# ViacheslavTimofeev/tpu_superresolution

Measured on AMD Instinct MI355X. Metric: HR pixels/sec, SwinIR x4 train step, 64x64 LR, bs=32/GPU, higher is better.
Workload: dtype bf16; 1 GPU; BASELINE cfg3: SwinIR classical x4 (dim 180, 6x6 blocks, window 8) train step = fwd + L1 + bwd + clip 1.0 + AdamW, 64x64 LR patches -> 256x256 HR, random-init weights, drop_path 0.1; every step starts from the seeded weights and fresh AdamW state; batch_per_gpu=32, global_batch=32, parallelism=dp1

## Files before the change

tpu_superresolution_amd/csrc/api.hip:

```cpp
#include <stdarg.h>
#include <stdio.h>
#include <string.h>

#include "adamw.h"
#include "kernels.h"
#include "tables.h"
#include "wgrad.h"

static thread_local char g_err[512] = "";

SrkOptTls& srk_opt_tls() {
  static thread_local SrkOptTls t = {};
  return t;
}

static SrkOpt** opt_table() {
  static SrkOpt* table[SRK_NUM_OPTS] = {};
  return table;
}

void srk_opt_register(SrkOpt* o) {
  if (o->id >= 0 && o->id < SRK_NUM_OPTS) opt_table()[o->id] = o;
}

// ... 320 lines not shown
  for (size_t i = 0; i < g_probe.count; ++i) {
    float t = 0.f;
    if (hipEventSynchronize(g_probe.ev1[i]) != hipSuccess || hipEventElapsedTime(&t, g_probe.ev0[i], g_probe.ev1[i]) != hipSuccess) {
      srk_set_error("probe_end: event query failed");
      return SRK_E_LAUNCH;
    }
    ms += t;
  }
  if (total_ms) *total_ms = ms;
  if (flops) *flops = g_probe.flops;
  if (bytes) *bytes = g_probe.bytes;
  if (launches) *launches = (int)g_probe.count;
  return SRK_OK;
}

namespace {

int tune_get(int which) {
  int v[4];
  srk_gemm_stream_tune_get(&v[0], &v[1], &v[2], &v[3]);
  return v[which];
}
int tune_set(int which, int value) {
  int v[4];
  srk_gemm_stream_tune_get(&v[0], &v[1], &v[2], &v[3]);
  v[which] = value;
  srk_gemm_stream_tune(v[0], v[1], v[2], v[3]);
  return SRK_OK;
}
int wtune_get(int which) {
  int rows, nt;
  srk_wgrad_stream_tune_get(&rows, &nt);
  return which == 0 ? rows : nt;
}

struct OptEntry {
  const char* name;
  int (*get)();
  int (*set)(int);
};

const OptEntry kOptions[] = {
    {"gemm_stream", [] { return srk_gemm_stream_enabled(); }, [](int v) { srk_gemm_stream_enable(v); return (int)SRK_OK; }},
    {"attn_bwd_fused", [] { return srk_attn_bwd_fused_enabled(); }, [](int v) { srk_attn_bwd_fused_enable(v); return (int)SRK_OK; }},
    {"attn_fused", [] { return srk_attn_fused_mode(); }, [](int v) { srk_attn_fused_enable(v); return (int)SRK_OK; }},
    {"wgrad_stream_w8", [] { return srk_wgrad_w8_enabled(); }, [](int v) { srk_wgrad_w8_enable(v); return (int)SRK_OK; }},
    {"block_light", [] { return srk_block_light_enabled(); }, [](int v) { srk_block_light_enable(v); return (int)SRK_OK; }},
    {"mlp_bwd_fused", [] { return srk_mlp_bwd_fused_enabled(); }, [](int v) { srk_mlp_bwd_fused_enable(v); return (int)SRK_OK; }},
    {"mlp_dgelu_store", [] { return srk_mlp_dgelu_store_enabled(); }, [](int v) { srk_mlp_dgelu_store_enable(v); return (int)SRK_OK; }},
    {"mlp_fused", [] { return srk_mlp_fused_enabled(); }, [](int v) { srk_mlp_fused_enable(v); return (int)SRK_OK; }},
    {"wgrad_stream", [] { return srk_wgrad_stream_enabled(); }, [](int v) { srk_wgrad_stream_enable(v); return (int)SRK_OK; }},
    {"conv_wgrad_taps", [] { return srk_conv_wgrad_taps_mode(); }, [](int v) { srk_conv_wgrad_taps_enable(v); return (int)SRK_OK; }},
    {"conv_wgrad_roll", [] { return srk_conv_wgrad_roll_enabled(); }, [](int v) { srk_conv_wgrad_roll_enable(v); return (int)SRK_OK; }},
    {"wgrad_partials", [] { return srk_wgrad_partials_enabled(); }, [](int v) { srk_wgrad_partials_enable(v); return (int)SRK_OK; }},
    {"wgrad_stream_rows", [] { return wtune_get(0); },
     [](int v) {
       SRK_REQUIRE(v == 32 || v == 64, SRK_E_SHAPE, "wgrad_stream_rows: 32/64");
       srk_wgrad_stream_tune(v, -1);
       return (int)SRK_OK;
     }},
    {"wgrad_stream_nt", [] { return wtune_get(1); }, [](int v) { srk_wgrad_stream_tune(0, v != 0); return (int)SRK_OK; }},
    {"gemm_stream_bm", [] { return tune_get(0); },
     [](int v) {
       SRK_REQUIRE(v == 0 || v == 16 || v == 32 || v == 64, SRK_E_SHAPE, "gemm_stream_bm: 0/16/32/64");
       return tune_set(0, v);
     }},
    {"gemm_stream_ks2", [] { return tune_get(1); }, [](int v) { return tune_set(1, v < 0 ? -1 : (v != 0)); }},
    {"gemm_stream_split", [] { return tune_get(2); }, [](int v) { return tune_set(2, v < 0 ? -1 : (v != 0)); }},
    {"gemm_stream_nb", [] { return tune_get(3); },
     [](int v) {
       SRK_REQUIRE(v == 0 || v == 4 || v == 8, SRK_E_SHAPE, "gemm_stream_nb: 0/4/8");
       return tune_set(3, v);
     }},
    {"probe_stride", [] { return g_probe.stride; },
     [](int v) {
       SRK_REQUIRE(v >= 1 && v <= 1024, SRK_E_SHAPE, "probe_stride: 1..1024");
       g_probe.stride = v;
       return (int)SRK_OK;
     }},
};

const OptEntry* find_option(const char* name) {
  for (const OptEntry& e : kOptions)
    if (strcmp(name, e.name) == 0) return &e;
  return nullptr;
}

}

int srk_set_option(const char* name, int value) {
  REQ_PTR(name);
  const OptEntry* e = find_option(name);
  if (!e) {
    srk_set_error("srk_set_option: unknown option '%s'", name);
    return SRK_E_UNSUPPORTED;
  }
  return e->set(value);
}

int srk_get_option(const char* name, int* value) {
  REQ_PTR(name); REQ_PTR(value);
  const OptEntry* e = find_option(name);
  if (!e) {
    srk_set_error("srk_get_option: unknown option '%s'", name);
    return SRK_E_UNSUPPORTED;
  }
// ... 402 lines not shown
```

tpu_superresolution_amd/csrc/common.h:

```cpp
#pragma once
#include <hip/hip_runtime.h>
#include <stdint.h>

#include "../../include/srk.h"

typedef unsigned short bf16_t;
typedef __attribute__((ext_vector_type(8))) short bf16x8_t;
typedef __attribute__((ext_vector_type(4))) short bf16x4_t;
typedef __attribute__((ext_vector_type(4))) float f32x4_t;

#define SRK_WAVE 64

void srk_set_error(const char* fmt, ...);
int srk_check_launch(const char* what);

constexpr int SRK_MAX_DEVICES = 64;
int srk_current_device();
int srk_device_cus();
enum SrkOptId {
  OPT_MLP_FUSED, OPT_MLP_BWD_FUSED, OPT_GEMM_STREAM, OPT_TUNE_BM, OPT_TUNE_KS2, OPT_TUNE_SPLIT, OPT_TUNE_NB, OPT_ATTN_BWD_FUSED,
  OPT_ATTN_FUSED, OPT_BLOCK_LIGHT, OPT_TAPS_ENABLED, OPT_TAPS_DMA, OPT_WGRAD_STREAM, OPT_WGRAD_ROWS, OPT_WGRAD_NT, OPT_WGRAD_W8,
  OPT_WGRAD_PARTIALS, OPT_MLP_DGELU_STORE, OPT_TAPS_ROLL, SRK_NUM_OPTS
};
struct SrkOptTls {
  int v[SRK_NUM_OPTS];
  unsigned on;
};
SrkOptTls& srk_opt_tls();
struct SrkOpt;
void srk_opt_register(SrkOpt* o);
void srk_opt_scope_begin(SrkOptTls* saved);
void srk_opt_scope_end(const SrkOptTls& saved);
struct SrkOpt {
  int id;
  int value;
  SrkOpt(int id_, int v) : id(id_), value(v) { srk_opt_register(this); }
  operator int() const {
    const SrkOptTls& t = srk_opt_tls();
    return ((t.on >> id) & 1u) ? t.v[id] : value;
  }
  SrkOpt& operator=(int v) {
    SrkOptTls& t = srk_opt_tls();
    if ((t.on >> id) & 1u) t.v[id] = v;
    else value = v;
    return *this;
  }
  SrkOpt(const SrkOpt&) = delete;
  SrkOpt& operator=(const SrkOpt&) = delete;
};

template <class T>
struct SrkPerDevice {
  T v[SRK_MAX_DEVICES] = {};
  T& here() { return v[srk_current_device()]; }
};

typedef SrkPerDevice<signed char> SrkLdsState;
int srk_reserve_lds_fn(const void* fn, int bytes, SrkLdsState& st, bool refuse_spills, const char* err_fmt, ...);
template <class K, class... A>
inline int srk_reserve_lds(K* kernel, size_t bytes, SrkLdsState& st, bool refuse_spills = false, const char* err_fmt = nullptr, A... a) {
  return srk_reserve_lds_fn(reinterpret_cast<const void*>(kernel), (int)bytes, st, refuse_spills, err_fmt, a...);
}

enum { FAM_GEMM_LINEAR = 1, FAM_GEMM_CONV = 2, FAM_WGRAD_LINEAR = 3, FAM_WGRAD_CONV = 4, FAM_ATTN_FWD = 5, FAM_ATTN_BWD = 6,
       FAM_LN = 7 };
void srk_probe_pre(int family, hipStream_t stream, double flops, double bytes = 0.0);
void srk_probe_post(int family, hipStream_t stream);

#define SRK_REQUIRE(cond, code, ...)      \
  do {                                    \
    if (!(cond)) {                        \
      srk_set_error(__VA_ARGS__);         \
      return (code);                      \
    }                                     \
  } while (0)
// ... 223 lines not shown
```

tpu_superresolution_amd/csrc/convwgrad.hip:

```cpp
#include <type_traits>

#include "wgrad.h"

#ifndef SRK_NT_TAPS
#define SRK_NT_TAPS 0
#endif

namespace {

constexpr int CT = 64;
constexpr int SP = 64 + 16;
constexpr int HALO = CT + 2;
constexpr int XROWS = 3 * HALO;
constexpr int YPIECES = CT * 8 / 256;
constexpr int XPIECES = (XROWS * 8 + 255) / 256;

template <bool SHUF>
__global__ __launch_bounds__(256) void conv_wgrad_taps_kernel(const WgradParams p, int ntiles, int chunks_per) {
  extern __shared__ __attribute__((aligned(16))) unsigned char smem[];
  bf16_t* Ys = reinterpret_cast<bf16_t*>(smem);
  bf16_t* Xs = Ys + 2 * CT * SP;

  const int tid = threadIdx.x, lane = tid & 63;
  const int wave = __builtin_amdgcn_readfirstlane(tid >> 6);
  const int r16 = lane & 15, g = lane >> 4;
  const int logical = xcd_remap(blockIdx.x, gridDim.x);
  const int bsplit = logical / ntiles, btile = logical - bsplit * ntiles;
  const int ntn = p.N / 64;
  const int tn = btile % ntn, tk = btile / ntn;
  const int n0 = tn * 64, k0 = tk * 64;
  const int c_begin = bsplit * chunks_per;
  const int c_end = min(p.M / CT, c_begin + chunks_per);
  if (c_begin >= c_end) return;
  const int hw = p.H * p.W;

  uint4 ry[YPIECES], rx[XPIECES];
  auto load_stage = [&](int ch) {
    const int m0 = ch * CT;
    const int b = m0 / hw, rem = m0 - b * hw;
    const int y = rem / p.W, x0 = rem - y * p.W;
#pragma unroll
    for (int t = 0; t < YPIECES; ++t) {
      const int pid = tid + 256 * t;
      const int row = pid >> 3, c8 = pid & 7;
      if constexpr (SHUF) {
        const int nn = n0 + c8 * 8;
        const int ij = nn / p.Cs, c = nn - ij * p.Cs;
        const int si = ij / p.r, sj = ij - si * p.r;
        ry[t] = *reinterpret_cast<const uint4*>(
            p.Y + (((long long)(b * p.H * p.r + y * p.r + si)) * (p.W * p.r) + (x0 + row) * p.r + sj) * p.Cs + c);
      } else {
        ry[t] = *reinterpret_cast<const uint4*>(p.Y + (long long)(m0 + row) * p.ldy + n0 + c8 * 8);
      }
    }
// ... 500 lines not shown
  const int cg = 9 * wave + q;
  const long long col = (long long)(cg >> 2) * p.K + tk * 64 + 16 * (cg & 3) + r16;
#pragma unroll
  for (int e = 0; e < 4; ++e) atomicAdd(p.dW + (long long)(n + e) * p.ldw + col, sum[e]);
}

SrkOpt g_taps_dma{OPT_TAPS_DMA, 1};
SrkOpt g_taps_roll{OPT_TAPS_ROLL, 1};

template <bool SHUF>
int launch_taps_dma(const WgradParams& p, hipStream_t stream) {
  constexpr int lds_staged = TD_RING * TD_STAGE_BYTES;
  constexpr int lds_roll = RL<2>::LDS > RL<1>::LDS ? RL<2>::LDS : RL<1>::LDS;
  static_assert(lds_roll <= 160 * 1024 && lds_staged <= 160 * 1024, "LDS budget");
  const int rpr = g_taps_roll && (p.W == CT || p.W == 2 * CT) && p.M % p.W == 0 ? p.W / CT : 0;
  static SrkLdsState reserved[2];
  constexpr const char* err = "conv wgrad (dma): cannot reserve %d bytes of LDS";
  constexpr int lds_max = lds_roll > lds_staged ? lds_roll : lds_staged;
  if (const int rc = rpr ? srk_reserve_lds(&conv_wgrad_taps_dma_kernel<SHUF>, lds_roll, reserved[1], false, err, lds_max)
                         : srk_reserve_lds(&conv_wgrad_taps_dma_staged_kernel<SHUF>, lds_staged, reserved[0], false, err, lds_max))
    return rc;
  const int lds = rpr == 1 ? RL<1>::LDS : (rpr == 2 ? RL<2>::LDS : lds_staged);
  const int unit = rpr ? rpr : 1;
  const int tiles = (p.N / 64) * (p.K / 64);
  const int nchunks = p.M / CT / unit;
  int splits = 256 / tiles;
  if (splits < 1) splits = 1;
  if (splits > nchunks) splits = nchunks;
  const int chunks_per = cdiv(nchunks, splits);
  splits = cdiv(nchunks, chunks_per);
  float* partial =
      srk_wgrad_partials_enabled() && splits > 1 ? srk_wgrad_scratch(stream, (size_t)tiles * splits * WS_SLAB_VEC * 16) : nullptr;
  srk_probe_pre(FAM_WGRAD_CONV, stream, p.flops, p.bytes);
  if (rpr)
    hipLaunchKernelGGL((conv_wgrad_taps_dma_kernel<SHUF>), dim3(tiles * splits), dim3(256), lds, stream, p, tiles, chunks_per * unit,
                       partial, splits, rpr);
  else
    hipLaunchKernelGGL((conv_wgrad_taps_dma_staged_kernel<SHUF>), dim3(tiles * splits), dim3(256), lds, stream, p, tiles, chunks_per,
                       partial, splits);
  if (partial) hipLaunchKernelGGL(conv_wgrad_taps_reduce_kernel, dim3(tiles * 36), dim3(256), 0, stream, p, partial, splits);
  srk_probe_post(FAM_WGRAD_CONV, stream);
  return srk_check_launch("conv wgrad (all taps, dma)");
}

__device__ __forceinline__ void split_bf16x8(const float (&v)[8], bf16x8_t& hi, bf16x8_t& lo) {
#pragma unroll
  for (int i = 0; i < 8; ++i) {
    const bf16_t h = f2bf(v[i]);
    hi[i] = (short)h;
    lo[i] = (short)f2bf(v[i] - bf2f(h));
  }
}

template <int COP>
struct SR {
  static constexpr int A = 3, NY = A + 1, NR = A + 3;
  static constexpr int GYB = CT * COP * 4;
  static constexpr int ROWB = HALO * 128;
  static constexpr int X_OFF = NY * GYB, Z_OFF = X_OFF + NR * ROWB, LDS = Z_OFF + ROWB;
};

template <bool NT = false>
__device__ __forceinline__ void srk_glds16_s1(const void* sb, unsigned voff, unsigned dst) {
  unsigned keep;
  asm volatile("s_mov_b32 %0, m0\n\ts_mov_b32 m0, %2\n\ts_nop 0\n\tglobal_load_lds_dwordx4 %1, %3\n\ts_mov_b32 m0, %0"
               : "=&s"(keep)
               : "v"(voff), "s"(dst), "s"(sb)
               : "memory");
}

__device__ __forceinline__ float lds_read_f32(unsigned addr) {
  return *reinterpret_cast<const float __attribute__((address_space(3)))*>(addr);
}

template <int COP>
__global__ __launch_bounds__(256, 2) void smallconv_wgrad_mfma_kernel(const bf16_t* __restrict__ x, const float* __restrict__ gy,
                                                                      float* __restrict__ dW, float* __restrict__ db, int B, int H, int W,
                                                                      int Cin, int CinP, int Co, int ntiles, int chunks_per) {
  using C = SR<COP>;
  extern __shared__ __attribute__((aligned(16))) unsigned char smem[];
  const unsigned lds0 = (unsigned)(size_t)smem;
  const int tid = threadIdx.x, lane = tid & 63;
  const int wave = __builtin_amdgcn_readfirstlane(tid >> 6);
  const int logical = xcd_remap(blockIdx.x, gridDim.x);
  const int bsplit = logical / ntiles, tk = logical - bsplit * ntiles;
  const int k0 = tk * 64;
  const int NCH = (int)(((long long)B * H * W) / CT);
  const int c_begin = bsplit * chunks_per;
  const int c_end = min(NCH, c_begin + chunks_per);
  if (c_begin >= c_end) return;
  const int nrun = c_end - c_begin;
  const int nxb = W / CT;
  for (int i = tid; i < HALO * 8; i += 256) *reinterpret_cast<uint4*>(smem + C::Z_OFF + i * 16) = make_uint4(0, 0, 0, 0);

  auto locate = [&](int ch, int& cy, int& cxb) -> long long {
    const int b = ch / (H * nxb), r = ch - b * (H * nxb);
    cxb = r / H;
    cy = r - cxb * H;
    return ((long long)(b * H + cy)) * W + cxb * CT;
  };
  auto step = [&](int& cy, int& cxb, const char*& ptr, long long ebytes) {
    if (++cy == H) {
      cy = 0;
      if (++cxb == nxb) {
        cxb = 0;
        ptr += CT * ebytes;
      } else {
        ptr += ((long long)CT - (long long)(H - 1) * W) * ebytes;
      }
    } else {
      ptr += (long long)W * ebytes;
    }
  };
  const long long xe = (long long)CinP * 2, ge = (long long)COP * 4;
  int xj = c_begin - 1, xy, xxb, gyy, gxb, y;
  const char* xptr = reinterpret_cast<const char*>(x + k0) + locate(max(xj, 0), xy, xxb) * xe;
  const char* gptr = reinterpret_cast<const char*>(gy) + locate(c_begin, gyy, gxb) * ge;
  y = gyy;
  const char* zero = reinterpret_cast<const char*>(g_zero_page);

  constexpr int LA = CT * COP / 16;
  const int l8 = lane >> 3, pos = lane & 7;
  const unsigned voffx = 2u * (unsigned)(l8 * CinP + ((((pos >> 1) ^ ((l8 >> 1) & 3)) << 1) | (pos & 1)) * 8);
  const unsigned voffh = (unsigned)(((wave & 1) * 4 + (lane & 3)) * 16);
  const unsigned voffg = (unsigned)((lane & (LA - 1)) * 16);
  const unsigned gdst0 = lds0 + (unsigned)(wave * LA * 16), gdst_end = gdst0 + C::NY * C::GYB;
  const unsigned xdst0 = lds0 + C::X_OFF, xdst_end = xdst0 + C::NR * C::ROWB;
  unsigned gdst = gdst0, xdst = xdst0;
  auto issue_y = [&]() {
    if (LA == 64 || lane < LA) srk_glds16_s1(gptr + wave * LA * 16, voffg, gdst);
    gdst = gdst + C::GYB == gdst_end ? gdst0 : gdst + C::GYB;
// ... 40 lines not shown
  for (int k = 0; k < C::A && k < nrun; ++k) {
    issue_y();
    issue_x();
  }
  const unsigned zrow = lds0 + C::Z_OFF;
  unsigned gs = lds0, xs0 = xdst0, xs1 = xdst0 + C::ROWB, xs2 = xdst0 + 2 * C::ROWB;
  auto run_loop = [&](auto bias) {
  constexpr bool BIAS = decltype(bias)::value;
  for (int it = 0; it < nrun; ++it) {
    if (it + C::A - 1 < nrun) srk_wait_vmcnt<4 * (C::A - 1)>(); else srk_wait_vmcnt<0>();
    srk_lds_barrier();
    if (it + C::A < nrun) {
      issue_y();
      issue_x();
    }
    const unsigned rb0 = y > 0 ? xs0 : zrow;
    const unsigned rb2 = y + 1 < H ? xs2 : zrow;
    const unsigned rbA = dA == 0 ? rb0 : (dA == 1 ? xs1 : rb2);
    const unsigned rbB = dB == 0 ? rb0 : (dB == 1 ? xs1 : rb2);
#pragma unroll
    for (int ks = 0; ks < 2; ++ks) {
      float v[8];
#pragma unroll
      for (int jj = 0; jj < 8; ++jj) {
        const float t = lds_read_f32(gs + goff + (unsigned)((32 * ks + 16 * (jj >> 2) + (jj & 3)) * COP * 4));
        v[jj] = ll < COP ? t : 0.f;
      }
      bf16x8_t yfh, yfl;
      split_bf16x8(v, yfh, yfl);
#pragma unroll
      for (int q = 0; q < 9; ++q) {
        const unsigned rb = q < nsel ? rbA : rbB;
        const bf16x4_t lo = lds_tr_read_at(ks == 0 ? rb + xoff0[q] : rb + (unsigned)xoff[q] + 32 * 128);
        const bf16x4_t hi = lds_tr_read_at(rb + (unsigned)xoff[q] + (32 * ks + 16) * 128);
        const bf16x8_t xf = bf16x8_t{lo[0], lo[1], lo[2], lo[3], hi[0], hi[1], hi[2], hi[3]};
        acc[q] = __builtin_amdgcn_mfma_f32_16x16x32_bf16(yfh, xf, acc[q], 0, 0, 0);
        acc[q] = __builtin_amdgcn_mfma_f32_16x16x32_bf16(yfl, xf, acc[q], 0, 0, 0);
      }
      if constexpr (BIAS) {
        accb = __builtin_amdgcn_mfma_f32_16x16x32_bf16(yfh, ones, accb, 0, 0, 0);
        accb = __builtin_amdgcn_mfma_f32_16x16x32_bf16(yfl, ones, accb, 0, 0, 0);
      }
    }
    gs = gs + C::GYB == lds0 + C::X_OFF ? lds0 : gs + C::GYB;
    xs0 = xs1;
    xs1 = xs2;
    xs2 = xs2 + C::ROWB == xdst_end ? xdst0 : xs2 + C::ROWB;
    y = y + 1 == H ? 0 : y + 1;
  }
  };
  if (do_bias) run_loop(std::true_type{});
  else run_loop(std::false_type{});

#pragma unroll
  for (int q = 0; q < 9; ++q) {
    const int cg = 9 * wave + q;
    const int tap = cg >> 2, k = k0 + 16 * (cg & 3) + ll;
#pragma unroll
    for (int e = 0; e < 4; ++e) {
      const int n = 4 * g + e;
      if (n < Co && k < Cin) atomicAdd(dW + ((long long)(n * Cin) + k) * 9 + tap, acc[q][e]);
    }
  }
  if (do_bias && ll == 0) {
#pragma unroll
    for (int e = 0; e < 4; ++e)
      if (4 * g + e < Co) atomicAdd(db + 4 * g + e, accb[e]);
  }
}

template <int COP>
__global__ __launch_bounds__(256) void smallconv_wgrad_mfma_staged_kernel(const bf16_t* __restrict__ x, const float* __restrict__ gy,
                                                                   float* __restrict__ dW, float* __restrict__ db, int B, int H, int W,
                                                                   int Cin, int CinP, int Co, int ntiles, int chunks_per) {
  extern __shared__ __attribute__((aligned(16))) unsigned char smem[];
  bf16_t* Yh = reinterpret_cast<bf16_t*>(smem);
  bf16_t* Yl = Yh + 2 * CT * 16;
  bf16_t* Xs = Yl + 2 * CT * 16;
  const int tid = threadIdx.x, lane = tid & 63;
  const int wave = __builtin_amdgcn_readfirstlane(tid >> 6);
  const int r16 = lane & 15, g = lane >> 4;
  const int logical = xcd_remap(blockIdx.x, gridDim.x);
  const int bsplit = logical / ntiles, tk = logical - bsplit * ntiles;
  const int k0 = tk * 64;
  const int M = B * H * W;
  const int c_begin = bsplit * chunks_per;
  const int c_end = min(M / CT, c_begin + chunks_per);
  if (c_begin >= c_end) return;
  const int hw = H * W;
  for (int i = tid; i < 2 * 2 * CT * 16 / 2; i += 256) reinterpret_cast<unsigned*>(Yh)[i] = 0u;

  constexpr int YP = CT * COP / 4;
  float4 ry = make_float4(0.f, 0.f, 0.f, 0.f);
  uint4 rx[XPIECES];
  const int nxb = W / CT;
  auto load_stage = [&](int ch) {
    const int b = ch / (H * nxb), r = ch - b * (H * nxb);
    const int xb = r / H, y = r - xb * H, x0 = xb * CT;
    const int m0 = b * hw + y * W + x0;
    if (tid < YP) ry = *reinterpret_cast<const float4*>(gy + (long long)m0 * COP + tid * 4);
#pragma unroll
    for (int t = 0; t < XPIECES; ++t) {
      const int pid = tid + 256 * t;
      const int hr = pid >> 3, c8 = pid & 7;
      const int rr = hr / HALO, px = hr - rr * HALO;
      const int yy = y + rr - 1, xx = x0 + px - 1;
// ... 39 lines not shown
    if (ch + 1 < c_end) load_stage(ch + 1);
    const bf16_t* yh = Yh + buf * CT * 16;
    const bf16_t* yl = Yl + buf * CT * 16;
    const bf16_t* xs = Xs + buf * XROWS * SP;
#pragma unroll
    for (int ks = 0; ks < 2; ++ks) {
      bf16x8_t yfh, yfl;
      {
        const bf16x4_t lo = lds_tr_read(tr_addr(yh, 16, 32 * ks + 4 * g, 0, lane));
        const bf16x4_t hi = lds_tr_read(tr_addr(yh, 16, 32 * ks + 16 + 4 * g, 0, lane));
        yfh = bf16x8_t{lo[0], lo[1], lo[2], lo[3], hi[0], hi[1], hi[2], hi[3]};
        const bf16x4_t lo2 = lds_tr_read(tr_addr(yl, 16, 32 * ks + 4 * g, 0, lane));
        const bf16x4_t hi2 = lds_tr_read(tr_addr(yl, 16, 32 * ks + 16 + 4 * g, 0, lane));
        yfl = bf16x8_t{lo2[0], lo2[1], lo2[2], lo2[3], hi2[0], hi2[1], hi2[2], hi2[3]};
      }
#pragma unroll
      for (int q = 0; q < 9; ++q) {
        const int cg = 9 * wave + q;
        const int tap = cg >> 2, kf = cg & 3;
        const int xb = (tap / 3) * HALO + (tap % 3);
        const bf16x4_t lo = lds_tr_read(tr_addr(xs, SP, xb + 32 * ks + 4 * g, 16 * kf, lane));
        const bf16x4_t hi = lds_tr_read(tr_addr(xs, SP, xb + 32 * ks + 16 + 4 * g, 16 * kf, lane));
        const bf16x8_t xf = bf16x8_t{lo[0], lo[1], lo[2], lo[3], hi[0], hi[1], hi[2], hi[3]};
        acc[q] = __builtin_amdgcn_mfma_f32_16x16x32_bf16(yfh, xf, acc[q], 0, 0, 0);
        acc[q] = __builtin_amdgcn_mfma_f32_16x16x32_bf16(yfl, xf, acc[q], 0, 0, 0);
      }
      if (do_bias) {
        accb = __builtin_amdgcn_mfma_f32_16x16x32_bf16(yfh, ones, accb, 0, 0, 0);
        accb = __builtin_amdgcn_mfma_f32_16x16x32_bf16(yfl, ones, accb, 0, 0, 0);
      }
    }
    if (ch + 1 < c_end) store_stage(buf ^ 1);
    __syncthreads();
  }

#pragma unroll
  for (int q = 0; q < 9; ++q) {
    const int cg = 9 * wave + q;
    const int tap = cg >> 2, k = k0 + 16 * (cg & 3) + r16;
#pragma unroll
    for (int e = 0; e < 4; ++e) {
      const int n = 4 * g + e;
      if (n < Co && k < Cin) atomicAdd(dW + ((long long)(n * Cin) + k) * 9 + tap, acc[q][e]);
    }
  }
  if (do_bias && r16 == 0) {
#pragma unroll
    for (int e = 0; e < 4; ++e)
      if (4 * g + e < Co) atomicAdd(db + 4 * g + e, accb[e]);
  }
}

template <int COP>
int launch_smallconv_mfma(const bf16_t* x, const float* gy, float* dW, float* db, int B, int H, int W, int Cin, int CinP, int Co,
                          hipStream_t stream) {
  constexpr int lds_staged = (int)((2 * 2 * CT * 16 + 2 * XROWS * SP) * sizeof(bf16_t));
  static_assert(2 * SR<COP>::LDS <= 160 * 1024, "two workgroups per CU");
  static SrkLdsState reserved[2];
  constexpr const char* err = "smallconv wgrad: cannot reserve %d bytes of LDS";
  constexpr int lds_max = SR<COP>::LDS > lds_staged ? SR<COP>::LDS : lds_staged;
  const bool roll = g_taps_roll;
  if (const int rc = roll ? srk_reserve_lds(&smallconv_wgrad_mfma_kernel<COP>, SR<COP>::LDS, reserved[1], false, err, lds_max)
                          : srk_reserve_lds(&smallconv_wgrad_mfma_staged_kernel<COP>, lds_staged, reserved[0], false, err, lds_max))
    return rc;
  const int tiles = CinP / 64;
  const int nchunks = (int)(((long long)B * H * W) / CT);
  int splits = 512 / tiles;
  if (splits > nchunks) splits = nchunks;
  const int chunks_per = cdiv(nchunks, splits);
  splits = cdiv(nchunks, chunks_per);
  if (roll)
    hipLaunchKernelGGL((smallconv_wgrad_mfma_kernel<COP>), dim3(tiles * splits), dim3(256), SR<COP>::LDS, stream, x, gy, dW, db, B, H, W,
                       Cin, CinP, Co, tiles, chunks_per);
  else
    hipLaunchKernelGGL((smallconv_wgrad_mfma_staged_kernel<COP>), dim3(tiles * splits), dim3(256), lds_staged, stream, x, gy, dW, db, B, H,
                       W, Cin, CinP, Co, tiles, chunks_per);
  return srk_check_launch("smallconv wgrad (mfma)");
}

__global__ __launch_bounds__(256) void imghead_dgrad_mfma_kernel(const float* __restrict__ gy, const float* __restrict__ wgt,
                                                                 bf16_t* __restrict__ dx, int B, int H, int W, int Cin, int Co, int nchunks) {
  constexpr int TP = 64 + 8;
  __shared__ __attribute__((aligned(16))) bf16_t T[64 * TP];
  const int tid = threadIdx.x, lane = tid & 63;
  const int wave = __builtin_amdgcn_readfirstlane(tid >> 6);
  const int r16 = lane & 15, g = lane >> 4;

  bf16x8_t wh[4][2], wl[4][2];
#pragma unroll
  for (int j = 0; j < 4; ++j)
#pragma unroll
    for (int ks = 0; ks < 2; ++ks) {
      float v[8];
#pragma unroll
      for (int jj = 0; jj < 8; ++jj) {
        const int k = 32 * ks + 8 * g + jj;
        const int tap = k >> 2, co = k & 3, ci = 16 * j + r16;
        v[jj] = (tap < 9 && co < Co && ci < Cin) ? wgt[((co * Cin) + ci) * 9 + tap] : 0.f;
      }
      split_bf16x8(v, wh[j][ks], wl[j][ks]);
    }

  const int hw = H * W;
  for (int c = blockIdx.x; c < nchunks; c += gridDim.x) {
    const int pix = c * 64 + 16 * wave + r16;
    const int b = pix / hw, rem = pix - b * hw;
    const int y = rem / W, x = rem - y * W;
    f32x4_t acc[4];
#pragma unroll
    for (int j = 0; j < 4; ++j) acc[j] = f32x4_t{0.f, 0.f, 0.f, 0.f};
#pragma unroll
    for (int ks = 0; ks < 2; ++ks) {
      float v[8];
#pragma unroll
      for (int half = 0; half < 2; ++half) {
        const int tap = 8 * ks + 2 * g + half;
        float4 gv = make_float4(0.f, 0.f, 0.f, 0.f);
        if (tap < 9) {
          const int yy = y - (tap / 3 - 1), xs = x - (tap % 3 - 1);
          if ((unsigned)yy < (unsigned)H && (unsigned)xs < (unsigned)W)
            gv = *reinterpret_cast<const float4*>(gy + ((long long)(b * H + yy) * W + xs) * 4);
        }
        v[4 * half] = gv.x; v[4 * half + 1] = gv.y; v[4 * half + 2] = gv.z; v[4 * half + 3] = gv.w;
      }
      bf16x8_t xh, xl;
      split_bf16x8(v, xh, xl);
#pragma unroll
      for (int j = 0; j < 4; ++j) {
        acc[j] = __builtin_amdgcn_mfma_f32_16x16x32_bf16(wh[j][ks], xh, acc[j], 0, 0, 0);
        acc[j] = __builtin_amdgcn_mfma_f32_16x16x32_bf16(wl[j][ks], xh, acc[j], 0, 0, 0);
        acc[j] = __builtin_amdgcn_mfma_f32_16x16x32_bf16(wh[j][ks], xl, acc[j], 0, 0, 0);
      }
    }
#pragma unroll
    for (int j = 0; j < 4; ++j)
      *reinterpret_cast<uint2*>(T + (16 * wave + r16) * TP + 16 * j + 4 * g) = pack_bf4(acc[j][0], acc[j][1], acc[j][2], acc[j][3]);
    srk_lds_barrier();
#pragma unroll
    for (int t = 0; t < 2; ++t) {
      const int pid = tid + 256 * t;
      const int row = pid >> 3, c8 = pid & 7;
      *reinterpret_cast<uint4*>(dx + ((long long)c * 64 + row) * 64 + c8 * 8) = *reinterpret_cast<const uint4*>(T + row * TP + c8 * 8);
    }
    srk_lds_barrier();
  }
}

}

void srk_conv_wgrad_taps_enable(int on) {
  g_taps_enabled = on ? 1 : 0;
  g_taps_dma = on >= 2 ? 1 : 0;
}
int srk_conv_wgrad_taps_mode() { return g_taps_enabled ? (g_taps_dma ? 2 : 1) : 0; }
void srk_conv_wgrad_roll_enable(int on) { g_taps_roll = on ? 1 : 0; }
int srk_conv_wgrad_roll_enabled() { return g_taps_roll; }

int srk_launch_conv_wgrad_taps(const WgradParams& p, hipStream_t stream) {
  if (!g_taps_enabled || !p.conv || p.W % CT != 0 || p.N % 64 != 0 || p.K % 64 != 0 || p.ldx % 8 != 0) return SRK_WGRAD_NOT_COVERED;
  if (p.r > 1) {
    if (p.Cs % 8 != 0 || p.N != p.r * p.r * p.Cs) return SRK_WGRAD_NOT_COVERED;
    return g_taps_dma ? launch_taps_dma<true>(p, stream) : launch_taps<true>(p, stream);
  }
  if (p.ldy % 8 != 0) return SRK_WGRAD_NOT_COVERED;
  return g_taps_dma ? launch_taps_dma<false>(p, stream) : launch_taps<false>(p, stream);
}

int srk_launch_smallconv_wgrad_mfma(const bf16_t* x, const float* gy, float* dW, float* db, int B, int H, int W, int Cin, int CinP,
                                    int Co, int CoP, hipStream_t stream) {
  if (!g_taps_enabled || W % CT != 0 || CinP % 64 != 0 || Co > CoP || ((long long)B * H * W) % CT != 0) return SRK_WGRAD_NOT_COVERED;
  if (CoP == 4) return launch_smallconv_mfma<4>(x, gy, dW, db, B, H, W, Cin, CinP, Co, stream);
  if (CoP == 16) return launch_smallconv_mfma<16>(x, gy, dW, db, B, H, W, Cin, CinP, Co, stream);
  return SRK_WGRAD_NOT_COVERED;
}

int srk_launch_imghead_dgrad_mfma(const float* gy, const float* wgt, bf16_t* dx, int B, int H, int W, int Cin, int CinP, int Co, int CoP,
                                  hipStream_t stream) {
  const long long npix = (long long)B * H * W;
  if (!g_taps_enabled || CoP != 4 || CinP != 64 || Co > 4 || Cin > 64 || npix % 64 != 0 || npix > (1ll << 30)) return SRK_WGRAD_NOT_COVERED;
  const int nchunks = (int)(npix / 64);
  const int grid = nchunks < 2048 ? nchunks : 2048;
  hipLaunchKernelGGL(imghead_dgrad_mfma_kernel, dim3(grid), dim3(256), 0, stream, gy, wgt, dx, B, H, W, Cin, Co, nchunks);
  return srk_check_launch("image-head dgrad (mfma)");
}
```

tpu_superresolution_amd/csrc/gemm.h:

```cpp
#pragma once
#include "common.h"

enum SrkLoader {
  LD_ROWS = 0,
  LD_CONV3 = 1,
  LD_CONV3_PS = 2,
};

enum SrkEpilogue {
  EP_BF16 = 0,
  EP_QKV = 1,
  EP_PROJ_RES = 2,
  EP_GELU = 3,
  EP_RES = 4,
  EP_DGELU = 5,
  EP_LRELU = 6,
  EP_PS = 7,
  EP_IMG = 8,
  EP_PS_IMG = 9,
  EP_RES_BF16 = 10,
  EP_DLRELU = 11,
  EP_F32_BF16 = 12,
  EP_LNBWD = 13,
};
// ... 1 lines not shown
struct GemmParams {
  const bf16_t* A;
  int lda;
  const bf16_t* Wt;
  int M, N, K;
  int B, H, W, CinP;
  int r, Cs;
  const float* bias;
  float* outf;
  bf16_t* outb;
  bf16_t* outb2;
  const float* res;
  const bf16_t* aux;
  double flops;
  double bytes;
  int ldo;
  float scale;
  int nH, CA;
  WinGeom geom;
  float inv_range;
  float mean[4];
  int Cimg, Hc, Wc;
  long long B_;
  const float* rowscale;
  int rows_per_sample;
  const float* ln_x;
  const float* ln_mean;
  const float* ln_rstd;
  const float* ln_gamma;
  float* ln_dgamma;
  float* ln_dbeta;
  int ln_C;
  int ln_rows_window, ln_stats_by_m, ln_out_window;
  float* ln_skip;
  bf16_t* xn_out;
  float* xn_mean;
  float* xn_rstd;
  const float* xn_gamma;
  const float* xn_beta;
  int xn_C, xn_window;
  WinGeom xn_geom;
  const bf16_t* W2;
  const float* bias2;
  bf16_t* u_out;
  int u_dgelu;
  bf16_t* h_out;
  int HP;
};

int srk_launch_gemm(int loader, int epilogue, const GemmParams& p, hipStream_t stream);

#define SRK_NOT_COVERED 1
int srk_launch_gemm_stream(int epilogue, const GemmParams& p, hipStream_t stream);
void srk_gemm_stream_enable(int on);
int srk_gemm_stream_enabled();
void srk_gemm_stream_tune_get(int* bm, int* ks2, int* split, int* nb);
void srk_gemm_stream_tune(int bm, int ks2, int split, int nb);
int srk_launch_mlp_fused(const GemmParams& p, hipStream_t stream);
void srk_mlp_fused_enable(int on);
int srk_mlp_fused_enabled();
int srk_launch_mlp_fused_bwd(const GemmParams& p, hipStream_t stream);
void srk_mlp_dgelu_store_enable(int on);
int srk_mlp_dgelu_store_enabled();
void srk_mlp_bwd_fused_enable(int on);
int srk_mlp_bwd_fused_enabled();
```

tpu_superresolution_amd/csrc/gemm.hip:

```cpp
#include "gemm.h"
#include "gemm_rowep.h"

namespace {

constexpr int BM = 128;
constexpr int BK = 64;

#ifndef SRK_GEMM_DMA
#define SRK_GEMM_DMA 1
#endif
__device__ uint4 g_gemm_zero[1];

template <int LD>
struct RowCtx {
  long long base[4];
  int yx[4];
};

template <int LD, int EP, int NT, bool NARROW>
__global__ __launch_bounds__(256) void gemm_kernel(const GemmParams p) {
  constexpr int BN = NARROW ? 16 : NT * 32;
  constexpr int WPASS = NARROW ? 1 : BN / 32;
  extern __shared__ __attribute__((aligned(16))) unsigned char smem[];
  bf16_t* As = reinterpret_cast<bf16_t*>(smem);
// ... 323 lines not shown
}

}

int srk_launch_gemm(int loader, int epilogue, const GemmParams& p, hipStream_t stream) {
  SRK_REQUIRE(p.M > 0 && p.N > 0 && p.K > 0 && p.K % BK == 0, SRK_E_SHAPE, "gemm: bad M/N/K %d/%d/%d", p.M, p.N, p.K);
  SRK_REQUIRE(p.A && p.Wt, SRK_E_NULL, "gemm: null operand");
  if (loader != LD_ROWS) {
    SRK_REQUIRE(p.CinP % 64 == 0 && p.K == 9 * p.CinP && p.M == p.B * p.H * p.W, SRK_E_SHAPE,
                "conv: inconsistent geometry K=%d CinP=%d M=%d B*H*W=%d", p.K, p.CinP, p.M, p.B * p.H * p.W);
    SRK_REQUIRE(p.H < 32768 && p.W < 32768, SRK_E_SHAPE, "conv: image too large");
    if (loader == LD_CONV3_PS) SRK_REQUIRE(p.Cs % 64 == 0 && p.CinP == p.r * p.r * p.Cs, SRK_E_SHAPE, "conv(ps-in): bad Cs");
  } else {
    SRK_REQUIRE(p.lda >= p.K && p.lda % 8 == 0, SRK_E_SHAPE, "gemm: bad lda %d", p.lda);
  }
  if (p.xn_out) {
    SRK_REQUIRE((epilogue == EP_PROJ_RES || epilogue == EP_RES) && (p.N == 64 || p.N == 128 || p.N == 192), SRK_E_SHAPE,
                "gemm: fused LayerNorm output needs a residual epilogue and N in {64,128,192} (N=%d)", p.N);
    SRK_REQUIRE(p.xn_mean && p.xn_rstd && p.xn_gamma && p.xn_beta, SRK_E_NULL, "gemm: fused LayerNorm: null pointer");
  }
  if (epilogue == EP_LNBWD) {
    SRK_REQUIRE(loader == LD_ROWS && (p.N == 64 || p.N == 128 || p.N == 192), SRK_E_SHAPE, "gemm(ln-bwd epilogue): N=%d must be one tile (64/128/192)", p.N);
    SRK_REQUIRE(p.ln_x && p.ln_mean && p.ln_rstd && p.ln_gamma && p.ln_dgamma && p.ln_dbeta && p.outf, SRK_E_NULL,
                "gemm(ln-bwd epilogue): null pointer");
  }
  if (loader == LD_ROWS) {
    const int rc = srk_launch_gemm_stream(epilogue, p, stream);
    if (rc != SRK_NOT_COVERED) return rc;
  }
#define CASE(LD, EP) \
  if (loader == LD && epilogue == EP) return dispatch_nt<LD, EP>(p, stream);
  CASE(LD_ROWS, EP_BF16)
  CASE(LD_ROWS, EP_QKV)
  CASE(LD_ROWS, EP_PROJ_RES)
  CASE(LD_ROWS, EP_GELU)
  CASE(LD_ROWS, EP_RES)
  CASE(LD_ROWS, EP_DGELU)
  CASE(LD_ROWS, EP_LNBWD)
  CASE(LD_ROWS, EP_LRELU)
  CASE(LD_ROWS, EP_DLRELU)
  CASE(LD_CONV3, EP_RES)
  CASE(LD_CONV3, EP_RES_BF16)
  CASE(LD_CONV3, EP_LRELU)
  CASE(LD_CONV3, EP_PS)
  CASE(LD_CONV3, EP_BF16)
  CASE(LD_CONV3, EP_DLRELU)
  CASE(LD_CONV3, EP_F32_BF16)
  CASE(LD_CONV3, EP_GELU)
  CASE(LD_CONV3, EP_DGELU)
  CASE(LD_ROWS, EP_RES_BF16)
  CASE(LD_CONV3_PS, EP_BF16)
  CASE(LD_CONV3_PS, EP_DLRELU)
#undef CASE
  if (loader == LD_CONV3 && epilogue == EP_IMG && p.N == 16) return launch<LD_CONV3, EP_IMG, 1, true>(p, stream);
  if (loader == LD_CONV3 && epilogue == EP_PS_IMG && p.N == 16) return launch<LD_CONV3, EP_PS_IMG, 1, true>(p, stream);
  srk_set_error("gemm: unsupported loader/epilogue combination %d/%d (N=%d)", loader, epilogue, p.N);
  return SRK_E_UNSUPPORTED;
}
```

Before: 76.97 million HR pixels/s.

## Add streaming image-head forward kernel, split-K partials for smallconv wgrad, prefetch dgrad

Adds a dedicated image-head forward conv kernel that streams row chunks into LDS with asynchronous global-to-LDS loads, keeping the weights in registers and using MFMA. It replaces the generic narrow GEMM path for the final 3x3 conv to the image channels. Separately, the small-conv weight-gradient kernel can now write per-split partials that a reduce kernel sums, avoiding many-way accumulation into dW. The image-head dgrad loop also prefetches the next chunk's gradient gathers. These are small stages of the step, so the overall effect is limited, and the extra reduce kernel and scratch memory add overhead.

```diff
diff --git a/tpu_superresolution_amd/csrc/api.hip b/tpu_superresolution_amd/csrc/api.hip
--- a/tpu_superresolution_amd/csrc/api.hip
+++ b/tpu_superresolution_amd/csrc/api.hip
@@ -396,6 +396,7 @@
     {"wgrad_stream", [] { return srk_wgrad_stream_enabled(); }, [](int v) { srk_wgrad_stream_enable(v); return (int)SRK_OK; }},
     {"conv_wgrad_taps", [] { return srk_conv_wgrad_taps_mode(); }, [](int v) { srk_conv_wgrad_taps_enable(v); return (int)SRK_OK; }},
     {"conv_wgrad_roll", [] { return srk_conv_wgrad_roll_enabled(); }, [](int v) { srk_conv_wgrad_roll_enable(v); return (int)SRK_OK; }},
+    {"imghead_fwd_stream", [] { return srk_imghead_fwd_stream_enabled(); }, [](int v) { srk_imghead_fwd_stream_enable(v); return (int)SRK_OK; }},
     {"wgrad_partials", [] { return srk_wgrad_partials_enabled(); }, [](int v) { srk_wgrad_partials_enable(v); return (int)SRK_OK; }},
     {"wgrad_stream_rows", [] { return wtune_get(0); },
      [](int v) {
diff --git a/tpu_superresolution_amd/csrc/common.h b/tpu_superresolution_amd/csrc/common.h
--- a/tpu_superresolution_amd/csrc/common.h
+++ b/tpu_superresolution_amd/csrc/common.h
@@ -20,7 +20,7 @@
 enum SrkOptId {
   OPT_MLP_FUSED, OPT_MLP_BWD_FUSED, OPT_GEMM_STREAM, OPT_TUNE_BM, OPT_TUNE_KS2, OPT_TUNE_SPLIT, OPT_TUNE_NB, OPT_ATTN_BWD_FUSED,
   OPT_ATTN_FUSED, OPT_BLOCK_LIGHT, OPT_TAPS_ENABLED, OPT_TAPS_DMA, OPT_WGRAD_STREAM, OPT_WGRAD_ROWS, OPT_WGRAD_NT, OPT_WGRAD_W8,
-  OPT_WGRAD_PARTIALS, OPT_MLP_DGELU_STORE, OPT_TAPS_ROLL, SRK_NUM_OPTS
+  OPT_WGRAD_PARTIALS, OPT_MLP_DGELU_STORE, OPT_TAPS_ROLL, OPT_IMGHEAD_FWD_STREAM, SRK_NUM_OPTS
 };
 struct SrkOptTls {
   int v[SRK_NUM_OPTS];
diff --git a/tpu_superresolution_amd/csrc/convwgrad.hip b/tpu_superresolution_amd/csrc/convwgrad.hip
--- a/tpu_superresolution_amd/csrc/convwgrad.hip
+++ b/tpu_superresolution_amd/csrc/convwgrad.hip
@@ -1,5 +1,6 @@
 #include <type_traits>
 
+#include "gemm.h"
 #include "wgrad.h"
 
 #ifndef SRK_NT_TAPS
@@ -606,6 +607,10 @@
   }
 }
 
+constexpr int SC_SLOTS = 37;
+template <int COP>
+constexpr int SC_LANES = COP == 4 ? 16 : 64;
+
 template <int COP>
 struct SR {
   static constexpr int A = 3, NY = A + 1, NR = A + 3;
@@ -630,7 +635,8 @@
 template <int COP>
 __global__ __launch_bounds__(256, 2) void smallconv_wgrad_mfma_kernel(const bf16_t* __restrict__ x, const float* __restrict__ gy,
                                                                       float* __restrict__ dW, float* __restrict__ db, int B, int H, int W,
-                                                                      int Cin, int CinP, int Co, int ntiles, int chunks_per) {
+                                                                      int Cin, int CinP, int Co, int ntiles, int chunks_per,
+                                                                      float* __restrict__ partial, int nsplit) {
   using C = SR<COP>;
   extern __shared__ __attribute__((aligned(16))) unsigned char smem[];
   const unsigned lds0 = (unsigned)(size_t)smem;
@@ -777,6 +783,16 @@
   if (do_bias) run_loop(std::true_type{});
   else run_loop(std::false_type{});
 
+  if (partial != nullptr) {
+    constexpr int LN = SC_LANES<COP>;
+    if (LN == 64 || g == 0) {
+      f32x4_t* slab = reinterpret_cast<f32x4_t*>(partial) + ((size_t)tk * nsplit + bsplit) * (SC_SLOTS * LN) + (LN == 64 ? lane : ll);
+#pragma unroll
+      for (int q = 0; q < 9; ++q) slab[(9 * wave + q) * LN] = acc[q];
+      if (wave == 0) slab[36 * LN] = accb;
+    }
+    return;
+  }
 #pragma unroll
   for (int q = 0; q < 9; ++q) {
     const int cg = 9 * wave + q;
@@ -922,6 +938,43 @@
 }
 
 template <int COP>
+__global__ __launch_bounds__(256) void smallconv_wgrad_reduce_kernel(const float* __restrict__ partial, float* __restrict__ dW,
+                                                                     float* __restrict__ db, int Cin, int Co, int nsplit) {
+  constexpr int LN = SC_LANES<COP>, NV = SC_SLOTS * LN;
+  __shared__ f32x4_t part[64][4];
+  const int tk = blockIdx.y;
+  const int vi = threadIdx.x & 3, sg = threadIdx.x >> 2;
+  const int v = blockIdx.x * 4 + vi;
+  const f32x4_t* src = reinterpret_cast<const f32x4_t*>(partial) + (size_t)tk * nsplit * NV + v;
+  f32x4_t sum = f32x4_t{0.f, 0.f, 0.f, 0.f};
+  for (int s0 = sg; s0 < nsplit; s0 += 64) sum += src[(size_t)s0 * NV];
+  part[sg][vi] = sum;
+  __syncthreads();
+#pragma unroll
+  for (int h = 32; h >= 1; h >>= 1) {
+    if (sg < h) part[sg][vi] += part[sg + h][vi];
+    __syncthreads();
+  }
+  if (sg != 0) return;
+  sum = part[0][vi];
+  const int t = v / LN, li = v - t * LN;
+  const int ll = li & 15, g = li >> 4;
+  if (t < 36) {
+    const int tap = t >> 2, k = tk * 64 + 16 * (t & 3) + ll;
+#pragma unroll
+    for (int e = 0; e < 4; ++e) {
+      const int n = 4 * g + e;
+      if (n < Co && k < Cin) dW[((long long)(n * Cin) + k) * 9 + tap] += sum[e];
+    }
+  } else if (tk == 0 && ll == 0 && db != nullptr) {
+#pragma unroll
+    for (int e = 0; e < 4; ++e)
+      if (4 * g + e < Co) db[4 * g + e] += sum[e];
+  }
+}
+
+
+template <int COP>
 int launch_smallconv_mfma(const bf16_t* x, const float* gy, float* dW, float* db, int B, int H, int W, int Cin, int CinP, int Co,
                           hipStream_t stream) {
   constexpr int lds_staged = (int)((2 * 2 * CT * 16 + 2 * XROWS * SP) * sizeof(bf16_t));
@@ -939,10 +992,15 @@
   if (splits > nchunks) splits = nchunks;
   const int chunks_per = cdiv(nchunks, splits);
   splits = cdiv(nchunks, chunks_per);
-  if (roll)
+  if (roll) {
+    constexpr int NV = SC_SLOTS * SC_LANES<COP>;
+    float* partial =
+        srk_wgrad_partials_enabled() && splits > 1 ? srk_wgrad_scratch(stream, (size_t)tiles * splits * NV * 16) : nullptr;
     hipLaunchKernelGGL((smallconv_wgrad_mfma_kernel<COP>), dim3(tiles * splits), dim3(256), SR<COP>::LDS, stream, x, gy, dW, db, B, H, W,
-                       Cin, CinP, Co, tiles, chunks_per);
-  else
+                       Cin, CinP, Co, tiles, chunks_per, partial, splits);
+    if (partial)
+      hipLaunchKernelGGL((smallconv_wgrad_reduce_kernel<COP>), dim3(NV / 4, tiles), dim3(256), 0, stream, partial, dW, db, Cin, Co, splits);
+  } else
     hipLaunchKernelGGL((smallconv_wgrad_mfma_staged_kernel<COP>), dim3(tiles * splits), dim3(256), lds_staged, stream, x, gy, dW, db, B, H,
                        W, Cin, CinP, Co, tiles, chunks_per);
   return srk_check_launch("smallconv wgrad (mfma)");
@@ -972,10 +1030,25 @@
     }
 
   const int hw = H * W;
-  for (int c = blockIdx.x; c < nchunks; c += gridDim.x) {
+  auto gather = [&](int c, float4 (&gv)[2][2]) {
     const int pix = c * 64 + 16 * wave + r16;
     const int b = pix / hw, rem = pix - b * hw;
     const int y = rem / W, x = rem - y * W;
+#pragma unroll
+    for (int ks = 0; ks < 2; ++ks)
+#pragma unroll
+      for (int half = 0; half < 2; ++half) {
+        const int tap = 8 * ks + 2 * g + half;
+        gv[ks][half] = make_float4(0.f, 0.f, 0.f, 0.f);
+        if (ks == 1 && half == 1) continue;
+        const int yy = y - (tap / 3 - 1), xs = x - (tap % 3 - 1);
+        const bool ok = tap < 9 && (unsigned)yy < (unsigned)H && (unsigned)xs < (unsigned)W;
+        const float4 t = *reinterpret_cast<const float4*>(gy + (ok ? ((long long)(b * H + yy) * W + xs) * 4 : 0ll));
+        if (ok) gv[ks][half] = t;
+      }
+  };
+  auto chunk = [&](int c, const float4 (&cur)[2][2], float4 (&nxt)[2][2]) {
+    gather(min(c + (int)gridDim.x, nchunks - 1), nxt);
     f32x4_t acc[4];
 #pragma unroll
     for (int j = 0; j < 4; ++j) acc[j] = f32x4_t{0.f, 0.f, 0.f, 0.f};
@@ -984,13 +1057,7 @@
       float v[8];
 #pragma unroll
       for (int half = 0; half < 2; ++half) {
-        const int tap = 8 * ks + 2 * g + half;
-        float4 gv = make_float4(0.f, 0.f, 0.f, 0.f);
-        if (tap < 9) {
-          const int yy = y - (tap / 3 - 1), xs = x - (tap % 3 - 1);
-          if ((unsigned)yy < (unsigned)H && (unsigned)xs < (unsigned)W)
-            gv = *reinterpret_cast<const float4*>(gy + ((long long)(b * H + yy) * W + xs) * 4);
-        }
+        const float4 gv = cur[ks][half];
         v[4 * half] = gv.x; v[4 * half + 1] = gv.y; v[4 * half + 2] = gv.z; v[4 * half + 3] = gv.w;
       }
       bf16x8_t xh, xl;
@@ -1013,8 +1080,166 @@
       *reinterpret_cast<uint4*>(dx + ((long long)c * 64 + row) * 64 + c8 * 8) = *reinterpret_cast<const uint4*>(T + row * TP + c8 * 8);
     }
     srk_lds_barrier();
-  }
-}
+  };
+  float4 ga[2][2], gb[2][2];
+  gather(blockIdx.x, ga);
+  for (int c = blockIdx.x; c < nchunks; c += 2 * gridDim.x) {
+    chunk(c, ga, gb);
+    if (c + (int)gridDim.x < nchunks) chunk(c + gridDim.x, gb, ga);
+  }
+}
+
+
+struct FR {
+  static constexpr int A = 4, NR = A + 3;
+  static constexpr int ROWB = HALO * 128;
+  static constexpr int Z_OFF = NR * ROWB, LDS = Z_OFF + ROWB;
+};
+
+__device__ __forceinline__ void srk_glds16_s2_nt(const void* sb0, const void* sb1, unsigned voff, unsigned dst0, unsigned dst1) {
+  unsigned keep;
+  asm volatile("s_mov_b32 %0, m0\n\ts_mov_b32 m0, %2\n\ts_nop 0\n\tglobal_load_lds_dwordx4 %1, %4 nt\n\ts_mov_b32 m0, %3\n\ts_nop 0\n\t"
+               "global_load_lds_dwordx4 %1, %5 nt\n\ts_mov_b32 m0, %0"
+               : "=&s"(keep)
+               : "v"(voff), "s"(dst0), "s"(dst1), "s"(sb0), "s"(sb1)
+               : "memory");
+}
+__device__ __forceinline__ void srk_glds16_s1_nt(const void* sb, unsigned voff, unsigned dst) {
+  unsigned keep;
+  asm volatile("s_mov_b32 %0, m0\n\ts_mov_b32 m0, %2\n\ts_nop 0\n\tglobal_load_lds_dwordx4 %1, %3 nt\n\ts_mov_b32 m0, %0"
+               : "=&s"(keep)
+               : "v"(voff), "s"(dst), "s"(sb)
+               : "memory");
+}
+__device__ __forceinline__ bf16x8_t lds_read_b128_at(unsigned addr) {
+  return *reinterpret_cast<const bf16x8_t __attribute__((address_space(3)))*>(addr);
+}
+
+__global__ __launch_bounds__(256, 2) void imghead_fwd_mfma_kernel(const GemmParams p, int chunks_per) {
+  using C = FR;
+  extern __shared__ __attribute__((aligned(16))) unsigned char smem[];
+  const unsigned lds0 = (unsigned)(size_t)smem;
+  const int tid = threadIdx.x, lane = tid & 63;
+  const int wave = __builtin_amdgcn_readfirstlane(tid >> 6);
+  const int r16 = lane & 15, g = lane >> 4;
+  const int H = p.H, W = p.W;
+  const int NCH = p.M / CT;
+  const int c_begin = blockIdx.x * chunks_per;
+  const int c_end = min(NCH, c_begin + chunks_per);
+  if (c_begin >= c_end) return;
+  const int nrun = c_end - c_begin;
+  const int nxb = W / CT;
+  for (int i = tid; i < HALO * 8; i += 256) *reinterpret_cast<uint4*>(smem + C::Z_OFF + i * 16) = make_uint4(0, 0, 0, 0);
+
+  bf16x8_t wf[9][2];
+#pragma unroll
+  for (int tap = 0; tap < 9; ++tap)
+#pragma unroll
+    for (int ks = 0; ks < 2; ++ks)
+      wf[tap][ks] = *reinterpret_cast<const bf16x8_t*>(p.Wt + (long long)r16 * p.K + tap * 64 + (ks * 4 + g) * 8);
+  float4 bv = make_float4(0.f, 0.f, 0.f, 0.f);
+  if (p.bias) bv = *reinterpret_cast<const float4*>(p.bias + 4 * g);
+
+  auto locate = [&](int ch, int& cb, int& cy, int& cxb) -> long long {
+    cb = ch / (H * nxb);
+    const int r = ch - cb * (H * nxb);
+    cxb = r / H;
+    cy = r - cxb * H;
+    return ((long long)(cb * H + cy)) * W + cxb * CT;
+  };
+  auto step = [&](int& cy, int& cxb, const char*& ptr, long long ebytes) {
+    if (++cy == H) {
+      cy = 0;
+      if (++cxb == nxb) {
+        cxb = 0;
+        ptr += CT * ebytes;
+      } else {
+        ptr += ((long long)CT - (long long)(H - 1) * W) * ebytes;
+      }
+    } else {
+      ptr += (long long)W * ebytes;
+    }
+  };
+  const long long xe = 128;
+  int xj = c_begin - 1, xb_, xy, xxb, ob, y, oxb;
+  const char* xptr = reinterpret_cast<const char*>(p.A) + locate(max(xj, 0), xb_, xy, xxb) * xe;
+  locate(c_begin, ob, y, oxb);
+  const char* zero = reinterpret_cast<const char*>(g_zero_page);
+
+  const int l8 = lane >> 3, pos = lane & 7;
+  const unsigned voffx = (unsigned)(l8 * 128 + ((pos ^ l8) << 4));
+  const unsigned voffh = (unsigned)(((((wave & 1) * 4 + (lane & 3)) ^ (wave >> 1)) << 4));
+  const unsigned xdst0 = lds0, xdst_end = xdst0 + C::NR * C::ROWB;
+  unsigned xdst = xdst0;
+  auto issue_x = [&]() {
+    const char* s = xptr + (long long)(wave * 16) * xe;
+    const unsigned d = xdst + (unsigned)(wave * 2048);
+    srk_glds16_s2_nt(s, s + 8 * xe, voffx, d, d + 1024);
+    const bool ok = wave < 2 ? xxb + 1 < nxb : xxb > 0;
+    const char* hb = ok ? (wave < 2 ? xptr + CT * xe : xptr - xe) : zero;
+    if (lane < 4) srk_glds16_s1_nt(hb, voffh, xdst + (unsigned)(CT * 128 + wave * 64));
+    xdst = xdst + C::ROWB == xdst_end ? xdst0 : xdst + C::ROWB;
+    ++xj;
+    if (xj > 0 && xj < NCH) step(xy, xxb, xptr, xe);
+  };
+
+  unsigned xoff[3][2];
+#pragma unroll
+  for (int dx = 0; dx < 3; ++dx) {
+    const int pr = 16 * wave + r16 + dx - 1;
+    const int p0 = pr < 0 ? HALO - 1 : pr;
+#pragma unroll
+    for (int ks = 0; ks < 2; ++ks) xoff[dx][ks] = (unsigned)(p0 * 128 + (((ks * 4 + g) ^ (p0 & 7)) << 4));
+  }
+
+  issue_x();
+  issue_x();
+  for (int k = 0; k < C::A && k < nrun; ++k) issue_x();
+  const unsigned zrow = lds0 + C::Z_OFF;
+  const long long plane = (long long)p.Hc * p.Wc;
+  unsigned xs0 = xdst0, xs1 = xdst0 + C::ROWB, xs2 = xdst0 + 2 * C::ROWB;
+  for (int it = 0; it < nrun; ++it) {
+    if (it + C::A - 1 < nrun) srk_wait_vmcnt<3 * (C::A - 1)>(); else srk_wait_vmcnt<0>();
+    srk_lds_barrier();
+    if (it + C::A < nrun) issue_x();
+    const unsigned rb0 = y > 0 ? xs0 : zrow;
+    const unsigned rb2 = y + 1 < H ? xs2 : zrow;
+    bf16x8_t xf[9][2];
+#pragma unroll
+    for (int tap = 0; tap < 9; ++tap) {
+      const unsigned rb = tap < 3 ? rb0 : (tap < 6 ? xs1 : rb2);
+#pragma unroll
+      for (int ks = 0; ks < 2; ++ks) xf[tap][ks] = lds_read_b128_at(rb + xoff[tap % 3][ks]);
+    }
+    __builtin_amdgcn_sched_barrier(0);
+    f32x4_t acc = f32x4_t{0.f, 0.f, 0.f, 0.f};
+#pragma unroll
+    for (int tap = 0; tap < 9; ++tap)
+#pragma unroll
+      for (int ks = 0; ks < 2; ++ks) acc = __builtin_amdgcn_mfma_f32_16x16x32_bf16(wf[tap][ks], xf[tap][ks], acc, 0, 0, 0);
+    const int x = oxb * CT + 16 * wave + r16;
+    if (g == 0 && y < p.Hc && x < p.Wc) {
+      float* o = p.outf + ((long long)ob * p.Cimg * plane + (long long)y * p.Wc + x);
+      const float vv[4] = {acc[0] + bv.x, acc[1] + bv.y, acc[2] + bv.z, acc[3] + bv.w};
+#pragma unroll
+      for (int e = 0; e < 4; ++e) {
+        if (e < p.Cimg) o[e * plane] = vv[e] * p.inv_range + p.mean[e];
+      }
+    }
+    xs0 = xs1;
+    xs1 = xs2;
+    xs2 = xs2 + C::ROWB == xdst_end ? xdst0 : xs2 + C::ROWB;
+    if (++y == H) {
+      y = 0;
+      if (++oxb == nxb) {
+        oxb = 0;
+        ++ob;
+      }
+    }
+  }
+}
+
+SrkOpt g_imghead_fwd_stream{OPT_IMGHEAD_FWD_STREAM, 1};
 
 }
 
@@ -1053,3 +1278,22 @@
   hipLaunchKernelGGL(imghead_dgrad_mfma_kernel, dim3(grid), dim3(256), 0, stream, gy, wgt, dx, B, H, W, Cin, Co, nchunks);
   return srk_check_launch("image-head dgrad (mfma)");
 }
+
+void srk_imghead_fwd_stream_enable(int on) { g_imghead_fwd_stream = on ? 1 : 0; }
+int srk_imghead_fwd_stream_enabled() { return g_imghead_fwd_stream; }
+
+int srk_launch_imghead_fwd(const GemmParams& p, hipStream_t stream) {
+  if (!g_imghead_fwd_stream || p.CinP != 64 || p.N != 16 || p.K != 9 * 64 || p.W % CT != 0 || p.Cimg > 4) return SRK_NOT_COVERED;
+  static SrkLdsState reserved;
+  if (const int rc = srk_reserve_lds(&imghead_fwd_mfma_kernel, FR::LDS, reserved, false, "image-head forward: cannot reserve %d bytes of LDS",
+                                     FR::LDS))
+    return rc;
+  const int nchunks = p.M / CT;
+  const int cus = srk_device_cus();
+  int chunks_per = cdiv(nchunks, 2 * (cus > 0 ? cus : 256));
+  if (chunks_per < 9) chunks_per = 9;
+  srk_probe_pre(FAM_GEMM_CONV, stream, p.flops, p.bytes);
+  hipLaunchKernelGGL(imghead_fwd_mfma_kernel, dim3(cdiv(nchunks, chunks_per)), dim3(256), FR::LDS, stream, p, chunks_per);
+  srk_probe_post(FAM_GEMM_CONV, stream);
+  return srk_check_launch("image-head forward (stream)");
+}
diff --git a/tpu_superresolution_amd/csrc/gemm.h b/tpu_superresolution_amd/csrc/gemm.h
--- a/tpu_superresolution_amd/csrc/gemm.h
+++ b/tpu_superresolution_amd/csrc/gemm.h
@@ -77,6 +77,9 @@
 
 #define SRK_NOT_COVERED 1
 int srk_launch_gemm_stream(int epilogue, const GemmParams& p, hipStream_t stream);
+int srk_launch_imghead_fwd(const GemmParams& p, hipStream_t stream);
+void srk_imghead_fwd_stream_enable(int on);
+int srk_imghead_fwd_stream_enabled();
 void srk_gemm_stream_enable(int on);
 int srk_gemm_stream_enabled();
 void srk_gemm_stream_tune_get(int* bm, int* ks2, int* split, int* nb);
diff --git a/tpu_superresolution_amd/csrc/gemm.hip b/tpu_superresolution_amd/csrc/gemm.hip
--- a/tpu_superresolution_amd/csrc/gemm.hip
+++ b/tpu_superresolution_amd/csrc/gemm.hip
@@ -399,7 +399,11 @@
   CASE(LD_CONV3_PS, EP_BF16)
   CASE(LD_CONV3_PS, EP_DLRELU)
 #undef CASE
-  if (loader == LD_CONV3 && epilogue == EP_IMG && p.N == 16) return launch<LD_CONV3, EP_IMG, 1, true>(p, stream);
+  if (loader == LD_CONV3 && epilogue == EP_IMG && p.N == 16) {
+    const int rc = srk_launch_imghead_fwd(p, stream);
+    if (rc != SRK_NOT_COVERED) return rc;
+    return launch<LD_CONV3, EP_IMG, 1, true>(p, stream);
+  }
   if (loader == LD_CONV3 && epilogue == EP_PS_IMG && p.N == 16) return launch<LD_CONV3, EP_PS_IMG, 1, true>(p, stream);
   srk_set_error("gemm: unsupported loader/epilogue combination %d/%d (N=%d)", loader, epilogue, p.N);
   return SRK_E_UNSUPPORTED;
```

Result: no change. 77.61 million HR pixels/s, median of 6 (+0.8%).
